# SDU-Gary/PCSS-Unet

Measured on AMD Instinct MI355X. Metric: frames/sec 7x512x512 U-Net fwd+bwd (train step), higher is better.
Workload: dtype f32; 1 GPU; configs[1]: batch=8/GPU 7x512x512 fp32 train step (fwd + 0.9*L1 + bwd + RCCL grad all-reduce + clip + AdamW); global_batch=8, in_ch=7, parallelism=dp1

## Files before the change

include/nsm.h:

```cpp
#ifndef NSM_H_
#define NSM_H_

#include <stddef.h>
#include <stdint.h>

#ifdef __cplusplus
extern "C" {
#endif

#define NSM_OK 0
#define NSM_E_ARG 1
#define NSM_E_HIP 2
#define NSM_E_WS 3

#define NSM_F32 0
#define NSM_BF16 1
#define NSM_F16 2

#define NSM_AMAX_WORDS 2048
#define NSM_PACK_FWD 0
#define NSM_PACK_DGRAD 1

int nsm_version(void);
int nsm_get_last_error(char* buf, size_t n);
// ... 71 lines not shown
int nsm_wino_gemm_f16m(const void* V, const void* U, int B, int H, int W, int cin_p, int cout_p,
                       int tile, void* M16, int* m16e, const uint32_t* amax_v, float beta_v,
                       const uint32_t* amax_u, float beta_u, void* stream);
int nsm_wino_output_bf16m(const void* M16, const int* m16e, int B, int H, int W, int cin_p,
                          int cout_p, int tile, const uint32_t* amax_v, float beta_v,
                          const uint32_t* amax_u, float beta_u, const float* bias, void* y, int ldy,
                          float* partial, int nslot, void* stream);
int nsm_wino_output_bf16m_act(const void* M16, const int* m16e, int B, int H, int W, int cin_p,
                              int cout_p, int tile, const uint32_t* amax_v, float beta_v,
                              const uint32_t* amax_u, float beta_u, const float* bias, void* y,
                              int ldy, const float* act_scale, const float* act_shift, float slope,
                              void* stream);
int nsm_wino_dout_f16(const void* dy, int lddy, int B, int H, int W, int c_p, int tile, void* dM,
                      const uint32_t* amax_dy, void* stream);
size_t nsm_wino_wgrad_f16_ws(int B, int H, int W, int cin_p, int cout_p, int tile);
int nsm_conv3x3_wgrad_wino_f16(const void* dM, const void* V, int B, int H, int W, int cin_p,
                               int cout_p, int cin, int cout, int tile, float* dw, float* ws,
                               size_t ws_floats, const uint32_t* amax_dy, const uint32_t* amax_x,
                               void* stream);
int nsm_wino_dual_input_bn_h2(const float* g, int ldg, const float* y, int ldy, int B, int H, int W,
                              int c_p, int tile, const float* scale, const float* shift,
                              float slope, const float* mask, const float* mean, const float* coef,
                              void* Vh, void* dMh, const uint32_t* bound, void* stream);
size_t nsm_wino_wgrad_h2_ws(int B, int H, int W, int cin_p, int cout_p, int tile);
int nsm_conv3x3_wgrad_wino_h2(const void* dMh, const void* Vh, int B, int H, int W, int cin_p,
                              int cout_p, int cin, int cout, int tile, float* dw, float* ws,
                              size_t ws_floats, const uint32_t* amax_dy, const uint32_t* amax_x,
                              void* stream);
int nsm_wino_gemm_h2(const void* V, const void* U, int B, int H, int W, int cin_p, int cout_p,
                     int tile, float* Mb, const uint32_t* amax_v, float beta_v,
                     const uint32_t* amax_u, float beta_u, void* stream);
int nsm_wino_gemm_h2_plan(int B, int H, int W, int cin_p, int cout_p, int tile, int* plan);
int nsm_wino_wgrad_h2_plan(int B, int H, int W, int cin_p, int cout_p, int tile, int* plan);
int nsm_wino_gemm_f16_plan(int B, int H, int W, int cin_p, int cout_p, int tile, int o16, int* plan);
int nsm_wino_wgrad_f16_plan(int B, int H, int W, int cin_p, int cout_p, int tile, int* plan);
int nsm_conv1x1_h2_rows(int M, int N, int K, int bnbwd);
int nsm_conv1x1_h2(const void* xh, int M, int cin_p, const void* wh, const float* bias, int cout_p,
                   float* y, int ldy, float* stats, const uint32_t* amax_x,
                   const uint32_t* amax_w, void* stream);
int nsm_conv1x1_dgrad_bnbwd_h2(const void* dy2h, int M, int cop, const void* w2dh, int cip,
                               const float* y1, int ldy1, const float* scale, const float* shift,
                               const float* mean, const float* invstd, const float* mask, int HW,
                               float slope, int mode, float* partial, const float* coef,
                               float* out, int ldo, const uint32_t* amax_dy2,
                               const uint32_t* amax_w, uint32_t* amax_out, uint32_t* amax_k1dz,
                               void* stream);
int nsm_set_h2d_bnb_persist(int form, int grid, int* prev);
int nsm_conv1x1_dgrad_bnbwd_h2_plan(int M, int cip, int cop, int* plan);
int nsm_h2d_tile_walk(int gx, int gy, int grid, int block, int* out, int cap, int* count);
size_t nsm_conv1x1_wgrad_h2_ws(int M, int cin_p, int cout_p);
int nsm_conv1x1_wgrad_h2(const void* dyh, const void* xh, int M, int cin_p, int cout_p, int cin,
                         int cout, float* dw, float* ws, size_t ws_floats, const uint32_t* amax_dy,
                         const uint32_t* amax_x, void* stream);
int nsm_conv3x3_h2_rows(int M, int N);
int nsm_conv3x3_h2(const void* xh, int B, int H, int W, int cin_p, const void* wh,
                   const float* bias, int cout_p, float* y, int ldy, float* stats,
                   const uint32_t* amax_x, const uint32_t* amax_w, void* stream);
size_t nsm_conv3x3_wgrad_h2_ws(int B, int H, int W, int cin_p, int cout_p);
int nsm_conv3x3_wgrad_h2(const void* dyh, const void* xh, int B, int H, int W, int cin_p,
                         int cout_p, int cin, int cout, float* dw, float* ws, size_t ws_floats,
                         const uint32_t* amax_dy, const uint32_t* amax_x, void* stream);
int nsm_set_f32_split(int mode);
int nsm_wino_output(const float* Mb, int B, int H, int W, int cout_p, int tile, const float* bias,
                    float* y, int ldy, void* stream);
int nsm_wino_output_stats(const float* Mb, int B, int H, int W, int cout_p, int tile,
                          const float* bias, float* y, int ldy, float* partial, int nslot,
// ... 348 lines not shown
```

pcss-unet_amd/csrc/nsm_conv_h2.hip:

```cpp
#include "nsm_conv.h"

namespace nsm_bf {
using namespace nsm;
#include "nsm_conv_s16_loaders.inc"
}

using namespace nsm;
using namespace nsm_bf;

#include "nsm_conv_h2.inc"
#include "nsm_conv_h2d.inc"

static bool h2_wg256() { static const bool v = env_flag("NSM_H2_WG256", true); return v; }

static void wino_wgrad_resplit(WinoWgradPlan& p, long long T, int cin_p, int cout_p, int nb,
                               long long target) {
  const long long tiles = (long long)ceil_div(cout_p, p.BM) * ceil_div(cin_p, p.BN) * nb;
  long long sp = (target + tiles - 1) / tiles, maxs = (T + 255) / 256;
  if (sp > maxs) sp = maxs;
  if (sp > 64) sp = 64;
  if (sp < 1) sp = 1;
  long long kc = (T + sp - 1) / sp;
  kc = (kc + BK - 1) / BK * BK;
  sp = (T + kc - 1) / kc;
// ... 15 lines not shown
  if (tiles >= cu_count()) sp = 1;
  if (sp > maxs) sp = maxs;
  if (sp > 64) sp = 64;
  if (sp < 1) sp = 1;
  long long kc = (T + sp - 1) / sp;
  kc = (kc + BK - 1) / BK * BK;
  sp = (T + kc - 1) / kc;
  if (tiles * sp < 768 && !(sp == 1 && tiles >= cu_count()))
    return plan_wino_wgrad(T, cin_p, cout_p, nb);
  p.splits = (int)sp;
  p.kchunk = (int)kc;
  p.slab_floats = (size_t)nb * sp * cout_p * cin_p;
  if (sp > 1) p.slab_floats += (size_t)nb * cout_p * cin_p;
  return p;
}

extern "C" size_t nsm_wino_wgrad_h2_ws(int B, int H, int W, int cin_p, int cout_p, int tile) {
  WinoGeom g;
  if (!wino_geom(tile, B, H, W, g)) return 0;
  return plan_wino_wgrad_h2(g.T, cin_p, cout_p, g.alpha2).slab_floats;
}

extern "C" int nsm_wino_wgrad_h2_plan(int B, int H, int W, int cin_p, int cout_p, int tile,
                                      int* plan) {
  WinoGeom g;
  NSM_CHECK_ARG(plan && wino_geom(tile, B, H, W, g) && cin_p > 0 && cout_p > 0 && cin_p % 32 == 0 &&
                    cout_p % 32 == 0,
                "wino_wgrad_h2_plan: bad args");
  const WinoWgradPlan p = plan_wino_wgrad_h2(g.T, cin_p, cout_p, g.alpha2);
  plan[0] = p.BM;
  plan[1] = p.BN;
  plan[2] = p.splits;
  plan[3] = p.kchunk;
  return 0;
}

extern "C" int nsm_conv3x3_wgrad_wino_h2(const void* dMh, const void* Vh, int B, int H, int W,
                                         int cin_p, int cout_p, int cin, int cout, int tile,
                                         float* dw, float* ws, size_t ws_floats,
                                         const uint32_t* amax_dy, const uint32_t* amax_x,
                                         void* stream) {
  NSM_CHECK_ARG(dMh && Vh && dw && ws && amax_dy && amax_x, "conv3x3_wgrad_wino_h2: null pointer");
  NSM_CHECK_ARG(cin_p % 32 == 0 && cout_p % 32 == 0 && cin <= cin_p && cout <= cout_p,
                "conv3x3_wgrad_wino_h2: bad channels");
  NSM_CHECK_ARG(((uintptr_t)dMh % 16) == 0 && ((uintptr_t)Vh % 16) == 0 && ((uintptr_t)ws % 16) == 0,
                "conv3x3_wgrad_wino_h2: alignment");
  WinoGeom g;
  NSM_CHECK_ARG(wino_geom(tile, B, H, W, g), "conv3x3_wgrad_wino_h2: bad tile or shape");
  const int nb = g.alpha2;
  WinoWgradPlan pl = plan_wino_wgrad_h2(g.T, cin_p, cout_p, nb);
  if (ws_floats < pl.slab_floats) return fail(NSM_E_WS, "conv3x3_wgrad_wino_h2: workspace too small");
  NSM_CHECK_ARG(g.T * 2 * (long long)std::max(cin_p, cout_p) < (1ll << 30),
                "conv3x3_wgrad_wino_h2: operand too large");
  hipStream_t s = as_stream(stream);
  const int M = cout_p, N = cin_p;
  const int rc = wino_wgrad_gemm_h2((const bf16_t*)dMh, (const bf16_t*)Vh, g.T, cin_p, cout_p, nb,
                                    pl.BM, pl.BN, pl.kchunk, pl.splits, ws,
                                    H2Scale{amax_dy, wino_beta(tile, 1)},
                                    H2Scale{amax_x, wino_beta(tile, 0)}, s);
  if (rc) return rc;
  return wgrad_wino_finish(ws, pl, nb, M, N, cin, cout, tile, dw, s);
}

extern "C" int nsm_to_h2(const float* x, int64_t rows, int C, const uint32_t* amax, float beta,
                         void* out, void* stream) {
  NSM_CHECK_ARG(x && out && amax && rows > 0 && C > 0 && C % 8 == 0 && beta > 0.f,
// ... 118 lines not shown
```

pcss-unet_amd/csrc/nsm_conv_h2.inc:

```


template <class E, class = void>
struct has_pre : std::false_type {};
template <class E>
struct has_pre<E, std::void_t<typename E::template PreT<1, 1>>> : std::true_type {};
template <class E, int TM, int TN, bool = has_pre<E>::value>
struct pre_of {
  struct type {};
};
template <class E, int TM, int TN>
struct pre_of<E, TM, TN, true> {
  using type = typename E::template PreT<TM, TN>;
};

struct H2RowsP {
  const bf16_t* x;
  int ld, nrows;
  long long bstride;
};
template <int R, int NW, int KT_ = 64>
struct H2RowsDma {
  static constexpr bool KM = false;
  static constexpr int KT = KT_;
  static constexpr int CH = KT / 8, RPI = 64 / CH;
// ... 181 lines not shown
    float* ob = e.out + (size_t)cx.zslab * e.bstride;
#pragma unroll
    for (int tm = 0; tm < TM; ++tm) {
#pragma unroll
      for (int tn = 0; tn < TN; ++tn)
#pragma unroll
        for (int i = 0; i < 16; ++i)
          reg[((i & 3) + 8 * (i >> 2) + 4 * h) * WCP + tn * 32 + col] = acc[tm][tn][i];
      __builtin_amdgcn_fence(__ATOMIC_RELEASE, "wavefront");
      __builtin_amdgcn_wave_barrier();
      __builtin_amdgcn_fence(__ATOMIC_ACQUIRE, "wavefront");
#pragma unroll
      for (int it = 0; it < 32 * CPR / 64; ++it) {
        const int q = it * 64 + cx.lane, r = q / CPR, cc = q - r * CPR;
        const int m = cx.mb + tm * 32 + r, n = cx.nb + cc * 4;
        if (m < M && n < N) *(f32x4*)(ob + (size_t)m * e.ld + n) = *(const f32x4*)&reg[r * WCP + cc * 4];
      }
      __builtin_amdgcn_fence(__ATOMIC_RELEASE, "wavefront");
      __builtin_amdgcn_wave_barrier();
      __builtin_amdgcn_fence(__ATOMIC_ACQUIRE, "wavefront");
    }
  }
};

template <int TM, int TN, class FA, class FB>
__device__ __forceinline__ void mfma_h2(f32x16 (&acc)[TM][TN], const FA (&fa)[2][TM],
                                        const FB (&fb)[2][TN], int tm, int tn) {
  f32x16 c = acc[tm][tn];
  c = __builtin_amdgcn_mfma_f32_32x32x16_f16(fa[1][tm].get(), fb[0][tn].get(), c, 0, 0, 0);
  c = __builtin_amdgcn_mfma_f32_32x32x16_f16(fa[0][tm].get(), fb[1][tn].get(), c, 0, 0, 0);
  acc[tm][tn] = __builtin_amdgcn_mfma_f32_32x32x16_f16(fa[0][tm].get(), fb[0][tn].get(), c, 0, 0, 0);
}

template <int BM, int BN, int WM, int WN, class AL, class BL, class EP, bool SP = false>
__global__ void __launch_bounds__(WM * WN * 64)
    gemm_h2_kernel(typename AL::P ap, typename BL::P bp, typename EP::P ep, int M, int N, int K,
                   int kchunk, int zsplit, int remap, H2Scale sca, H2Scale scb) {
  static_assert(!SP || (AL::KM && BL::KM), "single-plane: KM operands");
  constexpr int NPL = SP ? 1 : 2;
  constexpr int TM = BM / (WM * 32), TN = BN / (WN * 32);
  constexpr int A_EL = BM * 64, STAGE = (BM + BN) * 64;
  constexpr int KT = AL::KT;
  static_assert(KT == BL::KT, "K-tile");
  constexpr int LPT = AL::NI + BL::NI;
  constexpr int EPI = EP::template lds_bytes<TM, TN, WM, WN>() / 2;
  constexpr int LDS_EL = 2 * STAGE > EPI ? 2 * STAGE : EPI;
  __shared__ __attribute__((aligned(1024))) bf16_t lds[LDS_EL];

  const int tid = threadIdx.x, lane = tid & 63;
  const int wid = __builtin_amdgcn_readfirstlane(tid >> 6);
  const int wm = wid / WN, wn = wid % WN;
  int bx = blockIdx.x, by = blockIdx.y, bz = blockIdx.z;
  if (remap) xcd_block_order(bx, by, bz, remap);
  const int m0 = bx * BM, n0 = by * BN;
  const int split = bz % zsplit, batch = bz / zsplit;
  const int kbeg = split * kchunk;
  const int kend = min(K, kbeg + kchunk);
  const int nk = (kend - kbeg + KT - 1) / KT;
  const int ea = h2_exp(sca), eb = h2_exp(scb);
  const int kb0 = AL::KM ? 0 : kbeg;

  AL a;
  BL b;
  a.init(ap, m0, kbeg, kend, wid, lane, batch);
  b.init(bp, n0, kbeg, kend, wid, lane, batch);

  f32x16 acc[TM][TN];
#pragma unroll
  for (int i = 0; i < TM; ++i)
#pragma unroll
    for (int j = 0; j < TN; ++j)
#pragma unroll
      for (int e = 0; e < 16; ++e) acc[i][j][e] = 0.f;

  constexpr bool PRE = has_pre<EP>::value;
  typename pre_of<EP, TM, TN>::type pre;
  if constexpr (PRE)
    EP::template prefetch<TM, TN, WM, WN>(ep, pre, m0 + (wid / WN) * TM * 32,
                                          n0 + (wid % WN) * TN * 32, lane, M, N);

  if (nk > 0) {
    a.prep(ap, kb0);
    b.prep(bp, kb0);
#pragma unroll
    for (int j = 0; j < LPT; ++j) dma_one(a, b, ap, bp, lds, A_EL, wid, j);
  }
  if (nk > 1) {
    a.prep(ap, kb0 + KT);
    b.prep(bp, kb0 + KT);
#pragma unroll
    for (int j = 0; j < LPT; ++j) dma_one(a, b, ap, bp, lds + STAGE, A_EL, wid, j);
    vm_wait<LPT>();
  } else {
    vm_wait<0>();
  }
  dma_barrier();

  constexpr bool KMR = AL::KM || BL::KM;
  using FA = FragH2<AL::KM, AL::KM ? (SP ? BM : 2 * BM) : AL::KT, SP, sw2_of<AL>::value>;
  using FB = FragH2<BL::KM, BL::KM ? (SP ? BN : 2 * BN) : BL::KT, SP, sw2_of<BL>::value>;
  constexpr int NRT = NPL * (TM * FA::NR + TN * FB::NR);
  const int arb = wm * TM * 32, brb = wn * TN * 32;
  FA fa[2][2][TM];
  FB fb[2][2][TN];
#pragma unroll
  for (int p = 0; p < NPL; ++p) {
#pragma unroll
    for (int tm = 0; tm < TM; ++tm) fa[0][p][tm].issue(lds, arb + tm * 32, lane, 0, p);
#pragma unroll
    for (int tn = 0; tn < TN; ++tn) fb[0][p][tn].issue(lds + A_EL, brb + tn * 32, lane, 0, p);
  }
  constexpr int NS = AL::KM ? KT / 16 : 2;
  static_assert(NS == 2 || (NS == 4 && SP && AL::KM && BL::KM), "64-row K-tiles: single-plane KM");
  if constexpr (NS == 4) {
    for (int t = 0; t < nk; ++t) {
      const bf16_t* As = lds + (t & 1) * STAGE;
      const bf16_t* Bs = As + A_EL;
      const bool more = t + 1 < nk, refill = t + 2 < nk;
#pragma unroll
      for (int ks = 0; ks < NS; ++ks) {
        const int cur = ks & 1, nxt = cur ^ 1;
        if (ks + 1 < NS) {
#pragma unroll
          for (int tm = 0; tm < TM; ++tm) fa[nxt][0][tm].issue(As, arb + tm * 32, lane, ks + 1, 0);
#pragma unroll
          for (int tn = 0; tn < TN; ++tn) fb[nxt][0][tn].issue(Bs, brb + tn * 32, lane, ks + 1, 0);
          lgkm_fence_n<(NRT < 15 ? NRT : 15)>();
#pragma unroll
          for (int tm = 0; tm < TM; ++tm) fa[cur][0][tm].hold();
#pragma unroll
          for (int tn = 0; tn < TN; ++tn) fb[cur][0][tn].hold();
        } else {
          if (refill) {
            a.prep(ap, kb0 + (t + 2) * KT);
            b.prep(bp, kb0 + (t + 2) * KT);
          }
          __builtin_amdgcn_s_waitcnt(0xC07F);
          lgkm_fence();
#pragma unroll
          for (int tm = 0; tm < TM; ++tm) fa[cur][0][tm].hold();
#pragma unroll
          for (int tn = 0; tn < TN; ++tn) fb[cur][0][tn].hold();
          if (more) {
            vm_wait<0>();
            __builtin_amdgcn_s_barrier();
            const bf16_t* Ns = lds + ((t + 1) & 1) * STAGE;
#pragma unroll
            for (int tm = 0; tm < TM; ++tm) fa[nxt][0][tm].issue(Ns, arb + tm * 32, lane, 0, 0);
#pragma unroll
            for (int tn = 0; tn < TN; ++tn) fb[nxt][0][tn].issue(Ns + A_EL, brb + tn * 32, lane, 0, 0);
          }
        }
        __builtin_amdgcn_s_setprio(1);
#pragma unroll
        for (int tm = 0; tm < TM; ++tm)
#pragma unroll
          for (int tn = 0; tn < TN; ++tn) {
            acc[tm][tn] = __builtin_amdgcn_mfma_f32_32x32x16_f16(fa[cur][0][tm].get(), fb[cur][0][tn].get(),
                                                                 acc[tm][tn], 0, 0, 0);
            if (ks + 1 == NS && refill) {
              const int q = tm * TN + tn;
#pragma unroll
              for (int i = 0; i < LPT; ++i)
                if (i * (TM * TN) / LPT == q) dma_one(a, b, ap, bp, As, A_EL, wid, i);
            }
          }
        __builtin_amdgcn_s_setprio(0);
      }
    }
  } else
  for (int t = 0; t < nk; ++t) {
    const bf16_t* As = lds + (t & 1) * STAGE;
    const bf16_t* Bs = As + A_EL;
#pragma unroll
    for (int p = 0; p < NPL; ++p) {
#pragma unroll
      for (int tm = 0; tm < TM; ++tm) fa[1][p][tm].issue(As, arb + tm * 32, lane, 1, p);
#pragma unroll
      for (int tn = 0; tn < TN; ++tn) fb[1][p][tn].issue(Bs, brb + tn * 32, lane, 1, p);
    }
    if constexpr (KMR) {
      lgkm_fence_n<(NRT < 15 ? NRT : 15)>();
#pragma unroll
      for (int p = 0; p < NPL; ++p) {
#pragma unroll
        for (int tm = 0; tm < TM; ++tm) fa[0][p][tm].hold();
#pragma unroll
        for (int tn = 0; tn < TN; ++tn) fb[0][p][tn].hold();
      }
    }
    __builtin_amdgcn_s_setprio(1);
#pragma unroll
    for (int tm = 0; tm < TM; ++tm)
#pragma unroll
      for (int tn = 0; tn < TN; ++tn) {
        if constexpr (SP)
          acc[tm][tn] = __builtin_amdgcn_mfma_f32_32x32x16_f16(fa[0][0][tm].get(), fb[0][0][tn].get(),
                                                               acc[tm][tn], 0, 0, 0);
        else
          mfma_h2<TM, TN>(acc, fa[0], fb[0], tm, tn);
      }
    __builtin_amdgcn_s_setprio(0);
    const bool more = t + 1 < nk, refill = t + 2 < nk;
    if (refill) {
      a.prep(ap, kb0 + (t + 2) * KT);
      b.prep(bp, kb0 + (t + 2) * KT);
    }
    __builtin_amdgcn_s_waitcnt(0xC07F);
    if constexpr (KMR) {
      lgkm_fence();
#pragma unroll
      for (int p = 0; p < NPL; ++p) {
#pragma unroll
        for (int tm = 0; tm < TM; ++tm) fa[1][p][tm].hold();
#pragma unroll
        for (int tn = 0; tn < TN; ++tn) fb[1][p][tn].hold();
      }
    }
    if (more) {
      vm_wait<0>();
      __builtin_amdgcn_s_barrier();
      const bf16_t* Ns = lds + ((t + 1) & 1) * STAGE;
#pragma unroll
      for (int p = 0; p < NPL; ++p) {
#pragma unroll
        for (int tm = 0; tm < TM; ++tm) fa[0][p][tm].issue(Ns, arb + tm * 32, lane, 0, p);
#pragma unroll
        for (int tn = 0; tn < TN; ++tn) fb[0][p][tn].issue(Ns + A_EL, brb + tn * 32, lane, 0, p);
      }
    }
    __builtin_amdgcn_s_setprio(1);
#pragma unroll
    for (int tm = 0; tm < TM; ++tm)
#pragma unroll
      for (int tn = 0; tn < TN; ++tn) {
        if constexpr (SP)
          acc[tm][tn] = __builtin_amdgcn_mfma_f32_32x32x16_f16(fa[1][0][tm].get(), fb[1][0][tn].get(),
                                                               acc[tm][tn], 0, 0, 0);
        else
          mfma_h2<TM, TN>(acc, fa[1], fb[1], tm, tn);
        if (refill) {
          const int q = tm * TN + tn;
#pragma unroll
          for (int i = 0; i < LPT; ++i)
            if (i * (TM * TN) / LPT == q) dma_one(a, b, ap, bp, As, A_EL, wid, i);
        }
      }
    __builtin_amdgcn_s_setprio(0);
  }
  dma_barrier();
  const float ia = exp2i(-ea), ib = exp2i(-eb);
#pragma unroll
  for (int i = 0; i < TM; ++i)
#pragma unroll
    for (int j = 0; j < TN; ++j) acc[i][j] = (acc[i][j] * ia) * ib;
  EpiCtx cx{m0, n0, m0 + arb, n0 + brb, wm, wn, lane, (float*)lds, bx, bz};
  if constexpr (PRE) EP::template apply_pre<TM, TN, WM, WN>(ep, acc, cx, M, N, pre);
  else EP::template apply<TM, TN, WM, WN>(ep, acc, cx, M, N, split);
}


template <bool KM, int R, bool SP>
__device__ __forceinline__ f16x8 rd_h2q(const bf16_t* S, int rb, int p, int lane) {
  if constexpr (!KM) {
    const int row = rb + (lane & 15), chunk = 2 * (lane >> 4) + p;
    return __builtin_bit_cast(f16x8, *(const u32x4*)&S[row * R + ((chunk ^ dswz<R>(row)) << 3)]);
  } else {
    int ln = lane;
    asm volatile("" : "+v"(ln));
    const int q = (ln >> 2) & 3, pp = ln & 3, k = 8 * (ln >> 4) + q;
    const int c8 = (rb >> 3) + (pp >> 1), lc = SP ? c8 : 2 * c8 + p, sub = (pp & 1) * 4;
    typedef __attribute__((address_space(3))) s16x4 lds_s16x4;
    const s16x4 lo = __builtin_amdgcn_ds_read_tr16_b64_v4i16(
        (lds_s16x4*)(S + k * R + ((lc ^ kmswz2<R, SP>(k)) << 3) + sub));
    const s16x4 hi = __builtin_amdgcn_ds_read_tr16_b64_v4i16(
        (lds_s16x4*)(S + (k + 4) * R + ((lc ^ kmswz2<R, SP>(k + 4)) << 3) + sub));
    typedef short s16x8 __attribute__((ext_vector_type(8)));
    const s16x8 v = {lo.x, lo.y, lo.z, lo.w, hi.x, hi.y, hi.z, hi.w};
    return __builtin_bit_cast(f16x8, v);
  }
}
// ... 365 lines not shown
      for (int it = 0; it < 4; ++it) {
        const int r = it * 4 + (el >> 4), cc = el & 15;
        const f32x4 v = *(const f32x4*)&stg[r * 64 + ((4 * cc) ^ ((r >> 2) << 4))];
        const int m = m0 + arb + 16 * i + r, n = n0 + brb + 4 * cc;
        if constexpr (O16)
          __builtin_amdgcn_raw_buffer_store_b64(pack_f16x4(v), orsrc, (uint32_t)(m * ep.ld + n) * 2u,
                                                0, 0);
        else
          __builtin_amdgcn_raw_buffer_store_b128(__builtin_bit_cast(u32x4, v), orsrc,
                                                 (uint32_t)(m * ep.ld + n) * 4u, 0, 0);
      }
      __builtin_amdgcn_fence(__ATOMIC_RELEASE, "wavefront");
      __builtin_amdgcn_wave_barrier();
      __builtin_amdgcn_fence(__ATOMIC_ACQUIRE, "wavefront");
    }
    m0 = m0n;
    n0 = n0n;
    bz = bzn;
  }
}

__global__ void __launch_bounds__(256) to_h2_kernel(const float* __restrict__ x, long long rows,
                                                   int C, H2Scale sc, bf16_t* __restrict__ out) {
  const float s = exp2i(h2_exp(sc));
  const int C4 = C / 4;
  for (long long i = (long long)blockIdx.x * 256 + threadIdx.x; i < rows * C4;
       i += (long long)gridDim.x * 256) {
    const long long r = i / C4;
    const int c = (int)(i - r * C4) * 4;
    h2_store4(out + (size_t)r * 2 * C, c, *(const f32x4*)(x + (size_t)r * C + c), s);
  }
}

template <int BM, int BN, int WM, int WN, class AL, class BL>
static int launch_h2(dim3 grid, hipStream_t s, const typename AL::P& ap, const typename BL::P& bp,
                     const EpiH2P& ep, int M, int N, int K, int kchunk, int zsplit, H2Scale sa,
                     H2Scale sb) {
  constexpr int NT = WM * WN * 64;
  const long long total = (long long)grid.x * grid.y * grid.z;
  const int remap = split_xcd() && total % 8 == 0 && grid.z > 1 ? 1 : 0;
  hipLaunchKernelGGL((gemm_h2_kernel<BM, BN, WM, WN, AL, BL, EpiH2>), grid, dim3(NT), 0, s, ap, bp,
                     ep, M, N, K, kchunk, zsplit, remap, sa, sb);
  NSM_LAUNCH_CHECK("gemm_h2");
  return 0;
}

static bool h2_mf16() { static const bool v = env_flag("NSM_H2_MF16", true); return v; }

template <int BM, int BN, int WM, int WN, class AL, class BL, bool SP = false, bool O16 = false>
static int launch_h2q(dim3 grid, hipStream_t s, const typename AL::P& ap, const typename BL::P& bp,
                      const EpiH2P& ep, int M, int N, int K, H2Scale sa, H2Scale sb) {
  constexpr int NT = WM * WN * 64;
  const long long total = (long long)grid.x * grid.y * grid.z;
  const int remap = split_xcd() && total % 8 == 0 && grid.z > 1 ? 1 : 0;
  hipLaunchKernelGGL((gemm_h2q_kernel<BM, BN, WM, WN, AL, BL, SP, O16>), grid, dim3(NT), 0, s, ap, bp, ep,
                     M, N, K, K, 1, remap, sa, sb);
  NSM_LAUNCH_CHECK("gemm_h2q");
  return 0;
}

static bool h2p_nfast() { static const bool v = env_flag("NSM_H2P_NFAST", true); return v; }

static bool h2_persist() { static const bool v = env_flag("NSM_H2_PERSIST", true); return v; }

static bool h2_persistent(long long total, int K) {
  return h2_persist() && K % 128 == 0 && total > cu_count() && total < (1ll << 30);
}

template <int BM, int BN, int WM, int WN, class AL, class BL, bool SP = false, bool O16 = false>
static int launch_h2p(dim3 grid, hipStream_t s, const typename AL::P& ap, const typename BL::P& bp,
                      const EpiH2P& ep, int M, int N, int K, H2Scale sa, H2Scale sb) {
  constexpr int NT = WM * WN * 64;
  const long long total = (long long)grid.x * grid.y * grid.z;
  hipLaunchKernelGGL((gemm_h2p_kernel<BM, BN, WM, WN, AL, BL, SP, O16>), dim3(cu_count()), dim3(NT), 0, s,
                     ap, bp, ep, M, N, K, (int)grid.x, (int)grid.y, (int)total, sa, sb,
                     h2p_nfast() ? 1 : 0);
  NSM_LAUNCH_CHECK("gemm_h2p");
// ... 131 lines not shown
  if (wgrad_q()) {
    if (BM == 256 && BN == 256)
      return launch_h2qk<256, 256, 2, 4, F16PixDma<256, 8>, F16PixDma<256, 8>, true>(
          grid, s, ap, bp, ep, M, N, K, kchunk, splits, sdm, sv);
    if (BM == 128 && BN == 128)
      return launch_h2qk<128, 128, 2, 2, F16PixDma<128, 4>, F16PixDma<128, 4>, true>(
          grid, s, ap, bp, ep, M, N, K, kchunk, splits, sdm, sv);
    return fail(NSM_E_ARG, "wino_wgrad_gemm_f16: tile %dx%d", BM, BN);
  }
  if (BM == 256 && BN == 256 && f16_wg_kt64())
    hipLaunchKernelGGL((gemm_h2_kernel<256, 256, 2, 4, F16PixDma<256, 8, 64>, F16PixDma<256, 8, 64>, EpiH2,
                                       true>),
                       grid, dim3(512), 0, s, ap, bp, ep, M, N, K, kchunk, splits, remap, sdm, sv);
  else if (BM == 256 && BN == 256)
    hipLaunchKernelGGL((gemm_h2_kernel<256, 256, 2, 4, F16PixDma<256, 8>, F16PixDma<256, 8>, EpiH2, true>),
                       grid, dim3(512), 0, s, ap, bp, ep, M, N, K, kchunk, splits, remap, sdm, sv);
  else if (BM == 128 && BN == 128)
    hipLaunchKernelGGL((gemm_h2_kernel<128, 128, 2, 2, F16PixDma<128, 4>, F16PixDma<128, 4>, EpiH2, true>),
                       grid, dim3(256), 0, s, ap, bp, ep, M, N, K, kchunk, splits, remap, sdm, sv);
  else
    return fail(NSM_E_ARG, "wino_wgrad_gemm_f16: tile %dx%d", BM, BN);
  NSM_LAUNCH_CHECK("wino_wgrad_gemm_f16");
  return 0;
}

static int wino_wgrad_gemm_h2(const bf16_t* dM, const bf16_t* V, long long T, int cin_p,
                              int cout_p, int nb, int BM, int BN, int kchunk, int splits,
                              float* slab, H2Scale sdm, H2Scale sv, hipStream_t s) {
  const int M = cout_p, N = cin_p, K = (int)T;
  H2PixP ap{dM, 2 * cout_p, 2 * cout_p, (int)T, T * 2 * cout_p};
  H2PixP bp{V, 2 * cin_p, 2 * cin_p, (int)T, T * 2 * cin_p};
  EpiH2P ep{slab, N, (long long)M * N};
  const dim3 grid(ceil_div(M, BM), ceil_div(N, BN), nb * splits);
#define NSM_WH(bm, bn, wm, wn)                                                                   \
  if (BM == bm && BN == bn)                                                                      \
    return wgrad_q() ? launch_h2qk<bm, bn, wm, wn, H2PixDma<2 * bm, wm * wn>,                    \
                                   H2PixDma<2 * bn, wm * wn>>(grid, s, ap, bp, ep, M, N, K,      \
                                                              kchunk, splits, sdm, sv)           \
                     : launch_h2<bm, bn, wm, wn, H2PixDma<2 * bm, wm * wn>,                      \
                                 H2PixDma<2 * bn, wm * wn>>(grid, s, ap, bp, ep, M, N, K, kchunk, \
                                                            splits, sdm, sv);
  NSM_WH(256, 256, 2, 4)
  NSM_WH(128, 128, 2, 2)
  NSM_WH(128, 64, 2, 2)
  NSM_WH(64, 128, 2, 2)
  NSM_WH(64, 64, 2, 2)
  NSM_WH(128, 32, 4, 1)
  NSM_WH(32, 128, 1, 4)
  NSM_WH(64, 32, 2, 1)
  NSM_WH(32, 64, 1, 2)
#undef NSM_WH
  if (wgrad_q())
    return launch_h2qk<32, 32, 1, 1, H2PixDma<64, 1>, H2PixDma<64, 1>>(grid, s, ap, bp, ep, M, N, K,
                                                                     kchunk, splits, sdm, sv);
  return launch_h2<32, 32, 1, 1, H2PixDma<64, 1>, H2PixDma<64, 1>>(grid, s, ap, bp, ep, M, N, K,
                                                                   kchunk, splits, sdm, sv);
}
```

pcss-unet_amd/csrc/nsm_conv_h2d.inc:

```

struct EpiStoreH {
  using P = EpiStoreP;
  template <int TM, int TN, int WM, int WN>
  static constexpr int lds_bytes() {
    constexpr int a = WM * WN * 32 * (TN * 32 + 4) * 4, b = WM * WN * TN * 32 * 4;
    return a > b ? a : b;
  }
  template <int TM, int TN, int WM, int WN>
  __device__ static void apply(const P& e, f32x16 (&acc)[TM][TN], const EpiCtx& cx, int M, int N,
                               int) {
    const int col = cx.lane & 31, h = cx.lane >> 5;
#pragma unroll
    for (int tn = 0; tn < TN; ++tn) {
      const int n = cx.nb + tn * 32 + col;
      const float bv = (e.bias && n < N) ? e.bias[n] : 0.f;
#pragma unroll
      for (int tm = 0; tm < TM; ++tm)
#pragma unroll
        for (int i = 0; i < 16; ++i) acc[tm][tn][i] += bv;
    }
    constexpr int WC = TN * 32, WCP = WC + 4, CPR = WC / 4;
    float* reg = cx.lds + (cx.wm * WN + cx.wn) * (32 * WCP);
#pragma unroll
    for (int tm = 0; tm < TM; ++tm) {
// ... 486 lines not shown
  NSM_CHECK_ARG(plan && M > 0 && cip > 0 && cop > 0 && cip % 32 == 0 && cop % 32 == 0,
                "conv1x1_dgrad_bnbwd_h2_plan: bad args");
  const int K = 2 * cop, tile = h2d_tile(M, cip, K, true), bm = h2d_tile_bm(tile);
  const bool p = h2d_bnb_persistent(tile, M, cip, K, cip);
  const long long total = (long long)ceil_div(M, bm) * ceil_div(cip, 128);
  plan[0] = tile;
  plan[1] = p ? 1 : 0;
  plan[2] = !p ? 0 : tile == 2 ? h2bp_grid<256, 128, 4, 2>(total) : h2bp_grid<128, 128, 2, 2>(total);
  plan[3] = bm;
  return 0;
}

extern "C" int nsm_h2d_tile_walk(int gx, int gy, int grid, int block, int* out, int cap,
                                 int* count) {
  NSM_CHECK_ARG(out && count && gx > 0 && gy > 0 && grid > 0 && block >= 0 && block < grid &&
                    cap >= 0 && (long long)gx * gy < (1ll << 30),
                "h2d_tile_walk: bad args");
  int cnt = 0;
  for (int L = block; L < gx * gy; L += grid, ++cnt) {
    if (cnt >= cap) continue;
    int m, n;
    out[3 * cnt + 2] = h2d_tile_decode(L, gx, gy, m, n);
    out[3 * cnt] = m;
    out[3 * cnt + 1] = n;
  }
  *count = cnt;
  return 0;
}

extern "C" size_t nsm_conv1x1_wgrad_h2_ws(int M, int cin_p, int cout_p) {
  return plan_wgrad_h2(M, cin_p, cout_p).ws_floats;
}

extern "C" int nsm_conv1x1_wgrad_h2(const void* dyh, const void* xh, int M, int cin_p, int cout_p,
                                    int cin, int cout, float* dw, float* ws, size_t ws_floats,
                                    const uint32_t* amax_dy, const uint32_t* amax_x, void* stream) {
  NSM_CHECK_ARG(dyh && xh && dw && ws && amax_dy && amax_x, "conv1x1_wgrad_h2: null pointer");
  NSM_CHECK_ARG(M > 0 && cin_p % 32 == 0 && cout_p % 32 == 0 && cin <= cin_p && cout <= cout_p,
                "conv1x1_wgrad_h2: bad shape");
  NSM_CHECK_ARG(((uintptr_t)dyh % 16) == 0 && ((uintptr_t)xh % 16) == 0 && ((uintptr_t)ws % 16) == 0,
                "conv1x1_wgrad_h2: 16-B alignment");
  NSM_CHECK_ARG((long long)M * 2 * std::max(cin_p, cout_p) < (1ll << 30),
                "conv1x1_wgrad_h2: operand too large");
  const WgradPlan pl = plan_wgrad_h2(M, cin_p, cout_p);
  if (ws_floats < pl.ws_floats)
    return fail(NSM_E_WS, "conv1x1_wgrad_h2: workspace %zu < %zu floats", ws_floats, pl.ws_floats);
  hipStream_t s = as_stream(stream);
  const int rc = wino_wgrad_gemm_h2((const bf16_t*)dyh, (const bf16_t*)xh, M, cin_p, cout_p, 1,
                                    pl.BM, pl.BN, pl.kchunk, pl.splits, ws, H2Scale{amax_dy, 1.f},
                                    H2Scale{amax_x, 1.f}, s);
  if (rc) return rc;
  return wgrad_finish(ws, pl, cout_p, cin_p, cin_p, 1, cin, cout, dw, s);
}

template <int R, int NW>
struct H2ConvDma : ConvActDma<R, NW, 64> {
  static constexpr int KT = 64;
  __device__ void init(const ConvActPB& p, int m0, int kb, int ke, int wid, int lane, int) {
    ConvActDma<R, NW, 64>::init(p, m0, kb, ke, wid, lane);
  }
};
template <int R, int NW>
struct H2RowsKDma : RowsKDma<R, NW, 64> {
  static constexpr int KT = 64;
  __device__ void init(const RowsKPB& p, int n0, int kb, int ke, int wid, int lane, int) {
    RowsKDma<R, NW, 64>::init(p, n0, kb, ke, wid, lane);
// ... 128 lines not shown
```

pcss-unet_amd/nsm_amd/_lib.py:

```python
import ctypes
import os

import torch

_HERE = os.path.dirname(os.path.abspath(__file__))
LIB_PATH = os.environ.get("NSM_LIB", os.path.join(_HERE, "libnsm.so"))

P = ctypes.c_void_p
I = ctypes.c_int
L = ctypes.c_int64
F = ctypes.c_float
Z = ctypes.c_size_t
D = ctypes.c_double
U64 = ctypes.c_uint64

_SIGS = {
    "nsm_version": (I, []),
    "nsm_get_last_error": (I, [ctypes.c_char_p, Z]),
    "nsm_pack_conv_weight": (I, [P, I, I, I, I, I, I, P, P]),
    "nsm_pad_vec": (I, [P, I, I, P, P]),
    "nsm_conv_fwd": (I, [P, I, I, I, I, I, P, P, I, I, P, I, P, P, P, F, P]),
    "nsm_conv_stat_rows": (I, [I, I, I, I]),
    "nsm_conv_fwd_stats": (I, [P, I, I, I, I, I, P, P, I, I, P, I, P, P, P, F, P, P, P, P]),
    "nsm_wino_ws": (Z, [I, I, I, I, I, I]),
    "nsm_wino_weight": (I, [P, I, I, I, I, I, I, P, P]),
    "nsm_conv3x3_wino": (I, [P, I, I, I, I, I, P, P, I, I, I, P, I, P, Z, P]),
    "nsm_wino_input": (I, [P, I, I, I, I, I, I, I, P, P]),
    "nsm_wino_gemm": (I, [P, P, I, I, I, I, I, I, P, P]),
    "nsm_wino_gemm_s": (I, [P, P, I, I, I, I, I, I, P, P, P, P]),
    "nsm_absmax": (I, [P, L, P, P]),
    "nsm_zero_u32": (I, [P, L, P]),
    "nsm_absmax_bf16": (I, [P, L, P, P]),
    "nsm_pmc_calib": (I, [I, P, P, L, P]),
    "nsm_to_h2": (I, [P, L, I, P, F, P, P]),
    "nsm_wino_gemm_h2": (I, [P, P, I, I, I, I, I, I, P, P, F, P, F, P]),
    "nsm_wino_gemm_h2_plan": (I, [I, I, I, I, I, I, P]),
    "nsm_wino_wgrad_h2_plan": (I, [I, I, I, I, I, I, P]),
    "nsm_wino_gemm_f16_plan": (I, [I, I, I, I, I, I, I, P]),
    "nsm_wino_wgrad_f16_plan": (I, [I, I, I, I, I, I, P]),
    "nsm_wino_beta": (F, [I, I]),
    "nsm_wino_input_h2": (I, [P, I, I, I, I, I, I, I, I, P, P, P]),
    "nsm_wino_dual_input_h2": (I, [P, I, I, I, I, I, I, P, P, P, P]),
    "nsm_wino_dual_input_bn_h2": (I, [P, I, P, I, I, I, I, I, I, P, P, F, P, P, P, P, P, P, P]),
    "nsm_wino_input_f16": (I, [P, I, I, I, I, I, I, P, P, P]),
    "nsm_wino_input_f16_resize": (I, [P, I, I, I, I, I, I, I, I, P, P, P]),
    "nsm_wino_gemm_f16": (I, [P, P, I, I, I, I, I, I, P, P, F, P, F, P]),
    "nsm_wino_output_bf16": (I, [P, I, I, I, I, I, P, P, I, P, I, P]),
    "nsm_wino_gemm_f16m": (I, [P, P, I, I, I, I, I, I, P, P, P, F, P, F, P]),
    "nsm_wino_output_bf16m": (I, [P, P, I, I, I, I, I, I, P, F, P, F, P, P, I, P, I, P]),
    "nsm_wino_output_bf16m_act": (I, [P, P, I, I, I, I, I, I, P, F, P, F, P, P, I, P, P, F, P]),
    "nsm_wino_dout_f16": (I, [P, I, I, I, I, I, I, P, P, P]),
    "nsm_wino_dual_f16": (I, [P, I, I, I, I, I, I, P, P, P, P]),
    "nsm_wino_dual_bn_f16": (I, [P, I, P, I, I, I, I, I, I, P, P, F, P, P, P, P, P, P, P]),
    "nsm_wino_wgrad_f16_ws": (Z, [I, I, I, I, I, I]),
    "nsm_conv3x3_wgrad_wino_f16": (I, [P, P, I, I, I, I, I, I, I, I, P, P, Z, P, P, P]),
    "nsm_wino_wgrad_h2_ws": (Z, [I, I, I, I, I, I]),
    "nsm_conv3x3_wgrad_wino_h2": (I, [P, P, I, I, I, I, I, I, I, I, P, P, Z, P, P, P]),
    "nsm_set_f32_split": (I, [I]),
    "nsm_wino_output": (I, [P, I, I, I, I, I, P, P, I, P]),
    "nsm_wino_wgrad_ws": (Z, [I, I, I, I, I, I]),
    "nsm_conv3x3_wgrad_wino": (I, [P, I, P, I, I, I, I, I, I, I, I, P, P, Z, P]),
    "nsm_conv_wgrad_ws": (Z, [I, I, I, I, I, I]),
    "nsm_conv_wgrad": (I, [P, I, P, I, I, I, I, I, I, I, P, P, P, F, P, Z, I, I, P, P, P, P]),
    "nsm_reduce_chunks": (I, [I, I]),
    "nsm_reduce_rows": (I, [I, I]),
    "nsm_bn_stats": (I, [P, I, I, I, P, I, I, P]),
    "nsm_bn_finalize_train": (I, [P, I, I, I, I, I, P, P, P, P, P, F, F, I, P, P, P, P, P, F, P]),
    "nsm_bn_act_h2": (I, [P, I, I, I, P, P, F, P, I, P, P, P]),
    "nsm_conv1x1_h2_rows": (I, [I, I, I, I]),
    "nsm_conv1x1_h2": (I, [P, I, I, P, P, I, P, I, P, P, P, P]),
# ... 196 lines not shown
```

pcss-unet_amd/nsm_amd/ops.py:

```python
import os

import torch

from ._lib import call, ptr, stream

F32 = torch.float32
BF16 = torch.bfloat16
F16S = torch.int16
PACK_FWD, PACK_DGRAD = 0, 1
NSM_F32, NSM_BF16, NSM_F16 = 0, 1, 2
S16 = (BF16, F16S)


def dt(t):
    if t.dtype == BF16:
        return NSM_BF16
    if t.dtype == F16S:
        return NSM_F16
    if t.dtype != F32:
        raise TypeError(f"activations must be float32, bfloat16 or f16 storage (int16), "
                        f"got {t.dtype}")
    return NSM_F32


# ... 367 lines not shown
H2D_BNB_FORMS = ("policy", "old", "persistent")


def set_h2d_bnb_persist(form=-1, grid=-1):
    import ctypes
    if isinstance(form, str):
        form = H2D_BNB_FORMS.index(form)
    prev = (ctypes.c_int * 2)()
    call("nsm_set_h2d_bnb_persist", int(form), int(grid), prev)
    return prev[0], prev[1]


def conv1x1_dgrad_bnbwd_h2_plan(M, cip, cop):
    import ctypes
    plan = (ctypes.c_int * 4)()
    call("nsm_conv1x1_dgrad_bnbwd_h2_plan", M, cip, cop, plan)
    return plan[0], ("old", "persistent")[plan[1]], plan[2], plan[3]


def h2d_tile_walk(gx, gy, grid, block):
    import ctypes
    cap = -(-gx * gy // grid)
    out = (ctypes.c_int * (3 * max(cap, 1)))()
    cnt = ctypes.c_int(0)
    call("nsm_h2d_tile_walk", gx, gy, grid, block, out, cap, ctypes.byref(cnt))
    assert cnt.value <= cap
    return [(out[3 * i], out[3 * i + 1], out[3 * i + 2]) for i in range(cnt.value)]


def wino_wgrad_h2_plan(B, H, W, cin_p, cout_p, tile):
    import ctypes
    plan = (ctypes.c_int * 4)()
    call("nsm_wino_wgrad_h2_plan", B, H, W, cin_p, cout_p, tile, plan)
    return tuple(plan)


def wino_gemm_f16_plan(B, H, W, cin_p, cout_p, m16=False):
    import ctypes
    plan = (ctypes.c_int * 2)()
    call("nsm_wino_gemm_f16_plan", B, H, W, cin_p, cout_p, 4, int(bool(m16)), plan)
    return plan[0], H2_GEMM_FORMS[plan[1]]


def wino_wgrad_f16_plan(B, H, W, cin_p, cout_p):
    import ctypes
    plan = (ctypes.c_int * 4)()
    call("nsm_wino_wgrad_f16_plan", B, H, W, cin_p, cout_p, 4, plan)
    return tuple(plan)


def wino_dual_input_h2(dy, B, H, W, tile, amax_dy):
    c_p = dy.shape[1]
    n = (tile + 2) ** 2 * wino_tiles(B, H, W, tile) * 2 * c_p
    Vd = torch.empty(n, dtype=H2, device=dy.device)
    dM = torch.empty(n, dtype=H2, device=dy.device)
    call("nsm_wino_dual_input_h2", ptr(dy), dy.stride(0), B, H, W, c_p, tile, ptr(Vd), ptr(dM),
         ptr(amax_dy), stream())
    return Vd, dM


def wino_dual_input(dy, B, H, W, tile=4, amax=(None, None)):
    c_p = dy.shape[1]
    n = (tile + 2) ** 2 * wino_tiles(B, H, W, tile) * c_p
    Vd = empty(n, device=dy.device)
    dM = empty(n, device=dy.device)
    call("nsm_wino_dual_input", ptr(dy), dy.stride(0), B, H, W, c_p, tile, ptr(Vd), ptr(dM),
# ... 627 lines not shown
```

Baseline: 788.1 frames/s.

## Add configurable multi-stage LDS ring to fp16 wgrad GEMM kernel

Generalises the double-buffered LDS pipeline in the h2 GEMM kernel to an S-stage ring (up to 6), with partial vmcnt waits so more K-tiles stay in flight. A policy picks the ring depth per tile shape from LDS capacity, blocks per CU and a small table of shapes where deeper rings were preferred (64x32, and 128x128 at one block per CU). This is applied to Winograd and 1x1 weight-gradient launches to hide global-load latency in low-occupancy cases. Deeper rings use more LDS, which can lower occupancy, and each depth adds another compiled instantiation.

```diff
diff --git a/include/nsm.h b/include/nsm.h
--- a/include/nsm.h
+++ b/include/nsm.h
@@ -127,6 +127,10 @@
                      const uint32_t* amax_u, float beta_u, void* stream);
 int nsm_wino_gemm_h2_plan(int B, int H, int W, int cin_p, int cout_p, int tile, int* plan);
 int nsm_wino_wgrad_h2_plan(int B, int H, int W, int cin_p, int cout_p, int tile, int* plan);
+int nsm_set_h2_stages(int n, int* prev);
+int nsm_h2_ring_policy(int BM, int BN, int nk, long long blocks, int cus, int* plan);
+int nsm_wino_wgrad_h2_stages(int B, int H, int W, int cin_p, int cout_p, int tile, int* stages);
+int nsm_conv1x1_wgrad_h2_plan(int M, int cin_p, int cout_p, int* plan);
 int nsm_wino_gemm_f16_plan(int B, int H, int W, int cin_p, int cout_p, int tile, int o16, int* plan);
 int nsm_wino_wgrad_f16_plan(int B, int H, int W, int cin_p, int cout_p, int tile, int* plan);
 int nsm_conv1x1_h2_rows(int M, int N, int K, int bnbwd);
diff --git a/pcss-unet_amd/csrc/nsm_conv_h2.hip b/pcss-unet_amd/csrc/nsm_conv_h2.hip
--- a/pcss-unet_amd/csrc/nsm_conv_h2.hip
+++ b/pcss-unet_amd/csrc/nsm_conv_h2.hip
@@ -71,6 +71,38 @@
   plan[1] = p.BN;
   plan[2] = p.splits;
   plan[3] = p.kchunk;
+  return 0;
+}
+
+extern "C" int nsm_set_h2_stages(int n, int* prev) {
+  NSM_CHECK_ARG(n < 0 || n == 0 || (n >= 2 && n <= H2_RING_MAX), "set_h2_stages: %d", n);
+  if (prev) *prev = g_h2_stages;
+  if (n >= 0) g_h2_stages = n;
+  return 0;
+}
+
+extern "C" int nsm_h2_ring_policy(int BM, int BN, int nk, long long blocks, int cus, int* plan) {
+  NSM_CHECK_ARG(plan && nk >= 0 && blocks > 0 && cus > 0 &&
+                    (BM == 32 || BM == 64 || BM == 128 || BM == 256) &&
+                    (BN == 32 || BN == 64 || BN == 128 || BN == 256) && (BM == 256) == (BN == 256),
+                "h2_ring_policy: bad args");
+  const H2RingPlan p = h2_ring_policy(BM, BN, nk, blocks, cus);
+  plan[0] = p.S;
+  plan[1] = p.stage_bytes;
+  plan[2] = p.lpt;
+  plan[3] = p.per_cu;
+  plan[4] = h2_ring_cap(BM, BN);
+  return 0;
+}
+
+extern "C" int nsm_wino_wgrad_h2_stages(int B, int H, int W, int cin_p, int cout_p, int tile,
+                                        int* stages) {
+  WinoGeom g;
+  NSM_CHECK_ARG(stages && wino_geom(tile, B, H, W, g) && cin_p > 0 && cout_p > 0 &&
+                    cin_p % 32 == 0 && cout_p % 32 == 0,
+                "wino_wgrad_h2_stages: bad args");
+  const WinoWgradPlan p = plan_wino_wgrad_h2(g.T, cin_p, cout_p, g.alpha2);
+  *stages = wgrad_q() ? 2 : wgrad_h2_stages(cout_p, cin_p, g.T, g.alpha2, p.BM, p.BN, p.kchunk, p.splits);
   return 0;
 }
 
diff --git a/pcss-unet_amd/csrc/nsm_conv_h2.inc b/pcss-unet_amd/csrc/nsm_conv_h2.inc
--- a/pcss-unet_amd/csrc/nsm_conv_h2.inc
+++ b/pcss-unet_amd/csrc/nsm_conv_h2.inc
@@ -237,7 +237,7 @@
   acc[tm][tn] = __builtin_amdgcn_mfma_f32_32x32x16_f16(fa[0][tm].get(), fb[0][tn].get(), c, 0, 0, 0);
 }
 
-template <int BM, int BN, int WM, int WN, class AL, class BL, class EP, bool SP = false>
+template <int BM, int BN, int WM, int WN, class AL, class BL, class EP, bool SP = false, int S = 2>
 __global__ void __launch_bounds__(WM * WN * 64)
     gemm_h2_kernel(typename AL::P ap, typename BL::P bp, typename EP::P ep, int M, int N, int K,
                    int kchunk, int zsplit, int remap, H2Scale sca, H2Scale scb) {
@@ -249,7 +249,9 @@
   static_assert(KT == BL::KT, "K-tile");
   constexpr int LPT = AL::NI + BL::NI;
   constexpr int EPI = EP::template lds_bytes<TM, TN, WM, WN>() / 2;
-  constexpr int LDS_EL = 2 * STAGE > EPI ? 2 * STAGE : EPI;
+  static_assert(S >= 2 && S <= 6 && (S - 1) * LPT <= 63, "ring depth: vmcnt range");
+  static_assert(S * STAGE * 2 <= 160 * 1024, "ring depth: LDS");
+  constexpr int LDS_EL = S * STAGE > EPI ? S * STAGE : EPI;
   __shared__ __attribute__((aligned(1024))) bf16_t lds[LDS_EL];
 
   const int tid = threadIdx.x, lane = tid & 63;
@@ -284,20 +286,32 @@
     EP::template prefetch<TM, TN, WM, WN>(ep, pre, m0 + (wid / WN) * TM * 32,
                                           n0 + (wid % WN) * TN * 32, lane, M, N);
 
-  if (nk > 0) {
-    a.prep(ap, kb0);
-    b.prep(bp, kb0);
-#pragma unroll
-    for (int j = 0; j < LPT; ++j) dma_one(a, b, ap, bp, lds, A_EL, wid, j);
-  }
-  if (nk > 1) {
-    a.prep(ap, kb0 + KT);
-    b.prep(bp, kb0 + KT);
-#pragma unroll
-    for (int j = 0; j < LPT; ++j) dma_one(a, b, ap, bp, lds + STAGE, A_EL, wid, j);
-    vm_wait<LPT>();
+  if constexpr (S == 2) {
+    if (nk > 0) {
+      a.prep(ap, kb0);
+      b.prep(bp, kb0);
+#pragma unroll
+      for (int j = 0; j < LPT; ++j) dma_one(a, b, ap, bp, lds, A_EL, wid, j);
+    }
+    if (nk > 1) {
+      a.prep(ap, kb0 + KT);
+      b.prep(bp, kb0 + KT);
+#pragma unroll
+      for (int j = 0; j < LPT; ++j) dma_one(a, b, ap, bp, lds + STAGE, A_EL, wid, j);
+      vm_wait<LPT>();
+    } else {
+      vm_wait<0>();
+    }
   } else {
-    vm_wait<0>();
+#pragma unroll
+    for (int i = 0; i < S; ++i)
+      if (i < nk) {
+        a.prep(ap, kb0 + i * KT);
+        b.prep(bp, kb0 + i * KT);
+#pragma unroll
+        for (int j = 0; j < LPT; ++j) dma_one(a, b, ap, bp, lds + i * STAGE, A_EL, wid, j);
+      }
+    wait_retire<LPT, S - 1>(nk - 1);
   }
   dma_barrier();
 
@@ -317,6 +331,7 @@
   }
   constexpr int NS = AL::KM ? KT / 16 : 2;
   static_assert(NS == 2 || (NS == 4 && SP && AL::KM && BL::KM), "64-row K-tiles: single-plane KM");
+  static_assert(NS == 2 || S == 2, "64-row K-tiles: two stages");
   if constexpr (NS == 4) {
     for (int t = 0; t < nk; ++t) {
       const bf16_t* As = lds + (t & 1) * STAGE;
@@ -373,10 +388,12 @@
         __builtin_amdgcn_s_setprio(0);
       }
     }
-  } else
+  } else {
+  int slot = 0;
   for (int t = 0; t < nk; ++t) {
-    const bf16_t* As = lds + (t & 1) * STAGE;
+    const bf16_t* As = lds + (S == 2 ? (t & 1) : slot) * STAGE;
     const bf16_t* Bs = As + A_EL;
+    if constexpr (S > 2) slot = slot + 1 == S ? 0 : slot + 1;
 #pragma unroll
     for (int p = 0; p < NPL; ++p) {
 #pragma unroll
@@ -406,10 +423,10 @@
           mfma_h2<TM, TN>(acc, fa[0], fb[0], tm, tn);
       }
     __builtin_amdgcn_s_setprio(0);
-    const bool more = t + 1 < nk, refill = t + 2 < nk;
+    const bool more = t + 1 < nk, refill = t + S < nk;
     if (refill) {
-      a.prep(ap, kb0 + (t + 2) * KT);
-      b.prep(bp, kb0 + (t + 2) * KT);
+      a.prep(ap, kb0 + (t + S) * KT);
+      b.prep(bp, kb0 + (t + S) * KT);
     }
     __builtin_amdgcn_s_waitcnt(0xC07F);
     if constexpr (KMR) {
@@ -423,9 +440,9 @@
       }
     }
     if (more) {
-      vm_wait<0>();
+      wait_retire<LPT, S - 2>(nk - 2 - t);
       __builtin_amdgcn_s_barrier();
-      const bf16_t* Ns = lds + ((t + 1) & 1) * STAGE;
+      const bf16_t* Ns = lds + (S == 2 ? ((t + 1) & 1) : slot) * STAGE;
 #pragma unroll
       for (int p = 0; p < NPL; ++p) {
 #pragma unroll
@@ -452,6 +469,7 @@
         }
       }
     __builtin_amdgcn_s_setprio(0);
+  }
   }
   dma_barrier();
   const float ia = exp2i(-ea), ib = exp2i(-eb);
@@ -883,17 +901,97 @@
   }
 }
 
-template <int BM, int BN, int WM, int WN, class AL, class BL>
+template <int BM, int BN, int WM, int WN, class AL, class BL, int S = 2>
 static int launch_h2(dim3 grid, hipStream_t s, const typename AL::P& ap, const typename BL::P& bp,
                      const EpiH2P& ep, int M, int N, int K, int kchunk, int zsplit, H2Scale sa,
                      H2Scale sb) {
   constexpr int NT = WM * WN * 64;
   const long long total = (long long)grid.x * grid.y * grid.z;
   const int remap = split_xcd() && total % 8 == 0 && grid.z > 1 ? 1 : 0;
-  hipLaunchKernelGGL((gemm_h2_kernel<BM, BN, WM, WN, AL, BL, EpiH2>), grid, dim3(NT), 0, s, ap, bp,
-                     ep, M, N, K, kchunk, zsplit, remap, sa, sb);
+  hipLaunchKernelGGL((gemm_h2_kernel<BM, BN, WM, WN, AL, BL, EpiH2, false, S>), grid, dim3(NT), 0, s,
+                     ap, bp, ep, M, N, K, kchunk, zsplit, remap, sa, sb);
   NSM_LAUNCH_CHECK("gemm_h2");
   return 0;
+}
+
+static int g_h2_stages = [] {
+  const long long v = env_int("NSM_H2_STAGES", 0);
+  return v >= 2 && v <= 6 ? (int)v : 0;
+}();
+
+constexpr int H2_LDS_BYTES = 160 * 1024;
+constexpr int H2_RING_MAX = 6;
+
+constexpr int h2_km_waves(int BM, int BN) {
+  return BM + BN == 512 ? 8 : BM + BN >= 128 ? 4 : BM + BN == 96 ? 2 : 1;
+}
+constexpr int h2_km_stage_bytes(int BM, int BN) { return (BM + BN) * 128; }
+constexpr int h2_km_lpt(int BM, int BN) { return h2_km_stage_bytes(BM, BN) / 1024 / h2_km_waves(BM, BN); }
+constexpr int h2_ring_cap(int BM, int BN) {
+  if (!((BM >= 64 && BN >= 64) || BM + BN == 96)) return 2;
+  int c = H2_LDS_BYTES / h2_km_stage_bytes(BM, BN);
+  while (c > 2 && (c - 1) * h2_km_lpt(BM, BN) > 63) --c;
+  return c > H2_RING_MAX ? H2_RING_MAX : c < 2 ? 2 : c;
+}
+
+static int h2_ring_measured(int BM, int BN, long long per_cu) {
+  if (BM == 64 && BN == 32) return 3;
+  if (BM == 128 && BN == 128 && per_cu <= 1) return 3;
+  return 2;
+}
+
+struct H2RingPlan {
+  int S, stage_bytes, lpt, per_cu;
+};
+static H2RingPlan h2_ring_policy(int BM, int BN, int nk, long long blocks, int cus) {
+  H2RingPlan pl{2, h2_km_stage_bytes(BM, BN), h2_km_lpt(BM, BN), 0};
+  const long long want = std::max<long long>(1, std::min<long long>(2, (blocks + cus - 1) / cus));
+  pl.per_cu = (int)std::min<long long>(want, H2_LDS_BYTES / (2ll * pl.stage_bytes));
+  const int cap = std::min(h2_ring_measured(BM, BN, want), h2_ring_cap(BM, BN));
+  long long best = (long long)pl.per_cu * pl.stage_bytes;
+  for (int S = 3; S <= cap && S <= nk; ++S) {
+    if ((S - 2) * pl.lpt > 63) break;
+    const long long fit = H2_LDS_BYTES / ((long long)S * pl.stage_bytes);
+    if (fit < want) break;
+    const long long fly = want * (S - 1) * pl.stage_bytes;
+    if (fly > best) {
+      best = fly;
+      pl.S = S;
+      pl.per_cu = (int)want;
+    }
+  }
+  return pl;
+}
+
+static int h2_ring_stages(int BM, int BN, int kchunk, long long blocks) {
+  if (g_h2_stages) return std::min(g_h2_stages, h2_ring_cap(BM, BN));
+  return h2_ring_policy(BM, BN, ceil_div(kchunk, 32), blocks, cu_count()).S;
+}
+
+static int wgrad_h2_stages(int cout_p, int cin_p, long long T, int nb, int BM, int BN, int kchunk,
+                           int splits) {
+  const long long blocks = (long long)ceil_div(cout_p, BM) * ceil_div(cin_p, BN) * nb * splits;
+  return h2_ring_stages(BM, BN, (int)std::min<long long>(kchunk, T), blocks);
+}
+
+template <int BM, int BN, int WM, int WN>
+static int launch_h2_km(int S, dim3 grid, hipStream_t s, const H2PixP& ap, const H2PixP& bp,
+                        const EpiH2P& ep, int M, int N, int K, int kchunk, int zsplit, H2Scale sa,
+                        H2Scale sb) {
+  using AL = H2PixDma<2 * BM, WM * WN>;
+  using BL = H2PixDma<2 * BN, WM * WN>;
+  static_assert(WM * WN == h2_km_waves(BM, BN), "waves of the KM tile");
+  constexpr int CAP = h2_ring_cap(BM, BN);
+#define NSM_RING(n)                                                                              \
+  if constexpr (CAP >= n)                                                                        \
+    if (S == n)                                                                                  \
+      return launch_h2<BM, BN, WM, WN, AL, BL, n>(grid, s, ap, bp, ep, M, N, K, kchunk, zsplit, sa, sb);
+  NSM_RING(3)
+  NSM_RING(4)
+  NSM_RING(5)
+  NSM_RING(6)
+#undef NSM_RING
+  return launch_h2<BM, BN, WM, WN, AL, BL>(grid, s, ap, bp, ep, M, N, K, kchunk, zsplit, sa, sb);
 }
 
 static bool h2_mf16() { static const bool v = env_flag("NSM_H2_MF16", true); return v; }
@@ -1091,14 +1189,14 @@
   H2PixP bp{V, 2 * cin_p, 2 * cin_p, (int)T, T * 2 * cin_p};
   EpiH2P ep{slab, N, (long long)M * N};
   const dim3 grid(ceil_div(M, BM), ceil_div(N, BN), nb * splits);
+  const int S = wgrad_h2_stages(cout_p, cin_p, T, nb, BM, BN, kchunk, splits);
 #define NSM_WH(bm, bn, wm, wn)                                                                   \
   if (BM == bm && BN == bn)                                                                      \
     return wgrad_q() ? launch_h2qk<bm, bn, wm, wn, H2PixDma<2 * bm, wm * wn>,                    \
                                    H2PixDma<2 * bn, wm * wn>>(grid, s, ap, bp, ep, M, N, K,      \
                                                               kchunk, splits, sdm, sv)           \
-                     : launch_h2<bm, bn, wm, wn, H2PixDma<2 * bm, wm * wn>,                      \
-                                 H2PixDma<2 * bn, wm * wn>>(grid, s, ap, bp, ep, M, N, K, kchunk, \
-                                                            splits, sdm, sv);
+                     : launch_h2_km<bm, bn, wm, wn>(S, grid, s, ap, bp, ep, M, N, K, kchunk,     \
+                                                    splits, sdm, sv);
   NSM_WH(256, 256, 2, 4)
   NSM_WH(128, 128, 2, 2)
   NSM_WH(128, 64, 2, 2)
diff --git a/pcss-unet_amd/csrc/nsm_conv_h2d.inc b/pcss-unet_amd/csrc/nsm_conv_h2d.inc
--- a/pcss-unet_amd/csrc/nsm_conv_h2d.inc
+++ b/pcss-unet_amd/csrc/nsm_conv_h2d.inc
@@ -542,6 +542,18 @@
   return plan_wgrad_h2(M, cin_p, cout_p).ws_floats;
 }
 
+extern "C" int nsm_conv1x1_wgrad_h2_plan(int M, int cin_p, int cout_p, int* plan) {
+  NSM_CHECK_ARG(plan && M > 0 && cin_p > 0 && cout_p > 0 && cin_p % 32 == 0 && cout_p % 32 == 0,
+                "conv1x1_wgrad_h2_plan: bad args");
+  const WgradPlan pl = plan_wgrad_h2(M, cin_p, cout_p);
+  plan[0] = pl.BM;
+  plan[1] = pl.BN;
+  plan[2] = pl.splits;
+  plan[3] = pl.kchunk;
+  plan[4] = wgrad_q() ? 2 : wgrad_h2_stages(cout_p, cin_p, M, 1, pl.BM, pl.BN, pl.kchunk, pl.splits);
+  return 0;
+}
+
 extern "C" int nsm_conv1x1_wgrad_h2(const void* dyh, const void* xh, int M, int cin_p, int cout_p,
                                     int cin, int cout, float* dw, float* ws, size_t ws_floats,
                                     const uint32_t* amax_dy, const uint32_t* amax_x, void* stream) {
diff --git a/pcss-unet_amd/nsm_amd/_lib.py b/pcss-unet_amd/nsm_amd/_lib.py
--- a/pcss-unet_amd/nsm_amd/_lib.py
+++ b/pcss-unet_amd/nsm_amd/_lib.py
@@ -36,6 +36,10 @@
     "nsm_wino_gemm_h2": (I, [P, P, I, I, I, I, I, I, P, P, F, P, F, P]),
     "nsm_wino_gemm_h2_plan": (I, [I, I, I, I, I, I, P]),
     "nsm_wino_wgrad_h2_plan": (I, [I, I, I, I, I, I, P]),
+    "nsm_set_h2_stages": (I, [I, P]),
+    "nsm_h2_ring_policy": (I, [I, I, I, L, I, P]),
+    "nsm_wino_wgrad_h2_stages": (I, [I, I, I, I, I, I, P]),
+    "nsm_conv1x1_wgrad_h2_plan": (I, [I, I, I, P]),
     "nsm_wino_gemm_f16_plan": (I, [I, I, I, I, I, I, I, P]),
     "nsm_wino_wgrad_f16_plan": (I, [I, I, I, I, I, I, P]),
     "nsm_wino_beta": (F, [I, I]),
diff --git a/pcss-unet_amd/nsm_amd/ops.py b/pcss-unet_amd/nsm_amd/ops.py
--- a/pcss-unet_amd/nsm_amd/ops.py
+++ b/pcss-unet_amd/nsm_amd/ops.py
@@ -423,6 +423,34 @@
     import ctypes
     plan = (ctypes.c_int * 4)()
     call("nsm_wino_wgrad_h2_plan", B, H, W, cin_p, cout_p, tile, plan)
+    return tuple(plan)
+
+
+def set_h2_stages(n=-1):
+    import ctypes
+    prev = ctypes.c_int(0)
+    call("nsm_set_h2_stages", int(n), ctypes.byref(prev))
+    return prev.value
+
+
+def h2_ring_policy(BM, BN, nk, blocks, cus=256):
+    import ctypes
+    plan = (ctypes.c_int * 5)()
+    call("nsm_h2_ring_policy", BM, BN, nk, blocks, cus, plan)
+    return tuple(plan)
+
+
+def wino_wgrad_h2_stages(B, H, W, cin_p, cout_p, tile):
+    import ctypes
+    s = ctypes.c_int(0)
+    call("nsm_wino_wgrad_h2_stages", B, H, W, cin_p, cout_p, tile, ctypes.byref(s))
+    return s.value
+
+
+def conv1x1_wgrad_h2_plan(M, cin_p, cout_p):
+    import ctypes
+    plan = (ctypes.c_int * 5)()
+    call("nsm_conv1x1_wgrad_h2_plan", M, cin_p, cout_p, plan)
     return tuple(plan)
 
 
```

New measurement: 788.0 frames/s. Within noise of the previous version (-0.0%).
